# CUHK-AIM-Group/Depth-Aware-Endoscopy-SR

Hardware: AMD Instinct MI355X
Metric: LR frames/sec fwd+bwd at x8 (128x160 LR) (higher is better)
Workload: dtype f32; 1 GPU; Kvasir x8 synthetic, batch=16 per GPU, fp32, DepthNet nb=16 nf=64 L=256 K=10 (BASELINE.json configs[1]); step = fwd + L1 + dynamic loss + bwd + Adam; global_batch=16, scale=8, parallelism=dp1, mode=train, device=cuda, full=False, hip_graph=False

## Files before the change

depth-aware-endoscopy-sr_amd/csrc/bf16.h:

```cpp
#pragma once
#include "dasr_common.h"

typedef __bf16 bf16_t;
typedef __bf16 bf16x8 __attribute__((ext_vector_type(8)));
typedef __bf16 bf16x4 __attribute__((ext_vector_type(4)));
typedef short s16x4 __attribute__((ext_vector_type(4)));

#ifdef DASR_HIPEMU
static inline bf16_t dasr_f2bf(float f) {
    unsigned u;
    memcpy(&u, &f, 4);
    u = (u + 0x7FFFu + ((u >> 16) & 1u)) >> 16;
    unsigned short h = (unsigned short)u;
    bf16_t r;
    memcpy(&r, &h, 2);
    return r;
}
static inline float dasr_bf2f(bf16_t b) {
    unsigned short h;
    memcpy(&h, &b, 2);
    unsigned u = (unsigned)h << 16;
    float f;
    memcpy(&f, &u, 4);
    return f;
// ... 81 lines not shown
#ifdef DASR_HIPEMU
    const hipemu_s16x4 r = hipemu_ds_read_tr16_b64((const void*)p);
#else
    const s16x4 r = __builtin_amdgcn_ds_read_tr16_b64_v4i16((s16x4 __attribute__((address_space(3)))*)p);
#endif
    bf16x4 v;
    __builtin_memcpy(&v, &r, 8);
    return v;
}

typedef unsigned u32x4_t __attribute__((ext_vector_type(4)));
#define DASR_OOB 0x80000000u
#ifdef DASR_HIPEMU
struct BufRsrc {
    const char* base;
    size_t bytes;
};
static inline BufRsrc dasr_make_rsrc(const void* p, size_t bytes) { return BufRsrc{(const char*)p, bytes}; }
static inline u32x4_t dasr_buffer_load16(const BufRsrc& r, unsigned off) {
    u32x4_t v = {0u, 0u, 0u, 0u};
    if ((size_t)off + 16 <= r.bytes) memcpy(&v, r.base + off, 16);
    return v;
}
#else
typedef __amdgpu_buffer_rsrc_t BufRsrc;
__device__ __forceinline__ BufRsrc dasr_make_rsrc(const void* p, size_t bytes) {
    return __builtin_amdgcn_make_buffer_rsrc((void*)p, 0, (int)bytes, 0x00020000);
}
__device__ __forceinline__ u32x4_t dasr_buffer_load16(BufRsrc r, unsigned off) {
    return __builtin_amdgcn_raw_buffer_load_b128(r, (int)off, 0, 0);
}
#endif
```

depth-aware-endoscopy-sr_amd/csrc/conv9_split.hip:

```cpp
#include "bf16.h"
#include "conv_kernels.h"

typedef _Float16 h16_t;
typedef _Float16 h16x8 __attribute__((ext_vector_type(8)));
typedef _Float16 h16x4 __attribute__((ext_vector_type(4)));

#define S9_TH 8

struct Conv9SplitArgs {
    const float* x;
    const float* w;
    const float* bias;
    const float* dy;
    void* out;
    const float* xmax;
    const float* dmax;
    const float* wmax;
    int B, H, W, Cin, Cout;
    int accumulate, P, ntiles;
};

__device__ __forceinline__ float s9_amax_share(const float* buf) {
    float m = 0.f;
    if (buf) {
        int n;
        memcpy(&n, buf, 4);
        for (int i = threadIdx.x; i < n; i += blockDim.x) m = fmaxf(m, buf[1 + i]);
    }
#pragma unroll
    for (int o = 32; o > 0; o >>= 1) m = fmaxf(m, __shfl_xor(m, o));
    return m;
}
__host__ __device__ static inline int s9_scale_exp(float m) {
    unsigned u;
    memcpy(&u, &m, 4);
    int k = 14 - ((int)((u >> 23) & 0xffu) - 127);
    return k < -60 ? -60 : (k > 60 ? 60 : k);
}
__host__ __device__ static inline float s9_pow2(int k) {
    const unsigned u = (unsigned)(127 + k) << 23;
    float f;
    memcpy(&f, &u, 4);
// ... 178 lines not shown
            h16_t h0, h1;
            s9_split(8 * p8 + j < KK ? src[j] : 0.f, sd, h0, h1);
            o0[j] = h0; o1[j] = h1;
        }
        *(h16x8*)(sE0 + (row * S9_TQ + px) * EST + 8 * p8) = o0;
        *(h16x8*)(sE1 + (row * S9_TQ + px) * EST + 8 * p8) = o1;
    }
}
constexpr int S9_NDYE = (S9_TH + 8) * S9_DYW, S9_NDI = (S9_NDYE + 511) / 512;
__device__ __forceinline__ void s9_fetch_dy(const Conv9SplitArgs& a, int b, int y0, int x0, int tid, float (&vdy)[S9_NDI]) {
    const int rowf = (S9_TQ + 8) * a.Cout;
#pragma unroll
    for (int u = 0; u < S9_NDI; ++u) {
        const int idx = tid + 512 * u;
        const int f = idx % S9_DYW, ry = idx / S9_DYW;
        const int gy = y0 - 4 + ry, gx = x0 - 4 + f / a.Cout, co = f % a.Cout;
        const bool ok = idx < S9_NDYE && f < rowf && gy >= 0 && gy < a.H && gx >= 0 && gx < a.W;
        const size_t o = ok ? (((size_t)b * a.H + gy) * a.W + gx) * a.Cout + co : 0;
        const float v = a.dy[o];
        vdy[u] = ok ? v : 0.f;
    }
}

__global__ void __launch_bounds__(512) k_conv9_dgrad_split(Conv9SplitArgs a) {
    DASR_DYN_SMEM(smem);
    constexpr int EST = 40;
    constexpr int NE = (S9_TH + 8) * S9_TQ * EST;
    h16_t* sE0 = (h16_t*)smem;
    h16_t* sE1 = sE0 + NE;
    h16_t* sW0 = sE1 + NE;
    h16_t* sW1 = sW0 + 9 * 32 * EST;
    float* sDy = (float*)(sW1 + 9 * 32 * EST);
    float* s_red = sDy + S9_NDYE;
    const int tid = threadIdx.x, lane = tid & 63, wv = tid >> 6, li = lane & 31, lh = lane >> 5;
    const int tiles_x = (a.W + S9_TQ - 1) / S9_TQ, tiles_y = (a.H + S9_TH - 1) / S9_TH;
    const int total = tiles_x * tiles_y * a.B;
    const int n0 = blockIdx.y * 32;
    const int KK = 9 * a.Cout;
    int kd, kw_;
    s9_scales(a.dmax, a.wmax, s_red, kd, kw_);
    const float sd = s9_pow2(kd), sw = s9_pow2(kw_), inv = s9_pow2(-(kd + kw_));
    {
        float wq[18];
#pragma unroll
        for (int u = 0; u < 18; ++u) {
            const int e = tid + 512 * u, kp = e & 31, ci = (e >> 5) & 31, kh = e >> 10;
            const int kq = kp < KK ? kp : 0, kw = 8 - kq / a.Cout, co = kq % a.Cout;
            const float v = a.w[(((size_t)kh * 9 + kw) * a.Cin + n0 + ci) * a.Cout + co];
            wq[u] = kp < KK ? v : 0.f;
        }
#pragma unroll
        for (int u = 0; u < 18; ++u) {
            const int e = tid + 512 * u, kp = e & 31, ci = (e >> 5) & 31, kh = e >> 10;
            h16_t h0, h1;
            s9_split(wq[u], sw, h0, h1);
            sW0[(kh * 32 + ci) * EST + kp] = h0;
            sW1[(kh * 32 + ci) * EST + kp] = h1;
        }
    }
    float vdy[S9_NDI];
    auto origin = [&](int tile, int& b, int& x0, int& y0) {
        b = tile / (tiles_x * tiles_y);
        const int tt = tile - b * (tiles_x * tiles_y);
        x0 = (tt % tiles_x) * S9_TQ;
        y0 = (tt / tiles_x) * S9_TH;
    };
    int tile = blockIdx.x;
    if (tile < total) {
        int b, x0, y0;
        origin(tile, b, x0, y0);
        s9_fetch_dy(a, b, y0, x0, tid, vdy);
    }
    for (; tile < total; tile += gridDim.x) {
        int b, x0, y0;
        origin(tile, b, x0, y0);
        __syncthreads();
#pragma unroll
        for (int u = 0; u < S9_NDI; ++u) {
            const int idx = tid + 512 * u;
            if (idx < S9_NDYE) sDy[idx] = vdy[u];
        }
        __syncthreads();
        {
            int nb, nx0, ny0;
            origin(tile + (int)gridDim.x < total ? tile + (int)gridDim.x : tile, nb, nx0, ny0);
            s9_fetch_dy(a, nb, ny0, nx0, tid, vdy);
        }
        s9_build_E<EST>(a, sDy, sE0, sE1, sd, tid);
        __syncthreads();
        f32x16 acc;
#pragma unroll
        for (int r = 0; r < 16; ++r) acc[r] = 0.f;
#pragma unroll
        for (int kh = 0; kh < 9; ++kh)
#pragma unroll
            for (int q = 0; q < 2; ++q) {
                const int wo = (kh * 32 + li) * EST + 16 * q + 8 * lh;
                const h16x8 B0 = *(const h16x8*)(sW0 + wo), B1 = *(const h16x8*)(sW1 + wo);
                const int eo = ((wv - kh + 8) * S9_TQ + li) * EST + 16 * q + 8 * lh;
                const h16x8 A0 = *(const h16x8*)(sE0 + eo), A1 = *(const h16x8*)(sE1 + eo);
                acc = s9_mma(A0, A1, B0, B1, acc);
            }
        float* dx = (float*)a.out;
        const int gy = y0 + wv;
        if (gy < a.H) {
#pragma unroll
            for (int g = 0; g < 16; ++g) {
                const int gx = x0 + (g & 3) + 8 * (g >> 2) + 4 * lh;
                if (gx >= a.W) continue;
                const size_t o = (((size_t)b * a.H + gy) * a.W + gx) * a.Cin + n0 + li;
                float v = acc[g] * inv;
                if (a.accumulate) v += dx[o];
                dx[o] = v;
            }
        }
    }
}

__device__ __forceinline__ h16x4 s9_read_tr16(const h16_t* p) {
    const bf16x4 r = lds_read_tr16((const bf16_t*)p);
    h16x4 v;
    __builtin_memcpy(&v, &r, 8);
    return v;
}
__global__ void __launch_bounds__(512) k_conv9_wgrad_split(Conv9SplitArgs a) {
    DASR_DYN_SMEM(smem);
    constexpr int EST = 32;
    constexpr int NX = S9_TH * S9_TQ * 32, NE = (S9_TH + 8) * S9_TQ * EST;
    h16_t* sX0 = (h16_t*)smem;
    h16_t* sX1 = sX0 + NX;
    h16_t* sE0 = sX1 + NX;
    h16_t* sE1 = sE0 + NE;
    float* sDy = (float*)(sE1 + NE);
    float* s_red = sDy + S9_NDYE;
    const int tid = threadIdx.x, lane = tid & 63, wv = DASR_UNIFORM((int)(tid >> 6)), li = lane & 31, lh = lane >> 5;
    const int tiles_x = (a.W + S9_TQ - 1) / S9_TQ, tiles_y = (a.H + S9_TH - 1) / S9_TH;
    const int ci0 = blockIdx.x * 32;
    int kx, kd;
    s9_scales(a.xmax, a.dmax, s_red, kx, kd);
// ... 98 lines not shown
    const float* p = slabs + (size_t)(ci / 32) * (9 * 32 * 32) + (kh * 32 + (ci & 31)) * 32 + np;
    const int s0 = blockIdx.y * per_y;
    const int s1 = s0 + per_y < nslabs ? s0 + per_y : nslabs;
    float acc = 0.f;
    for (int s = s0; s < s1; ++s) acc += p[(size_t)s * cgroups * (9 * 32 * 32)];
    atomicAdd(&dw[i], acc);
}

bool conv9_split_supported(const ConvGeom& g) {
    return conv9_mfma_supported(g) && (g.Cin / 16) * 9 * 32 * S9F_ST * 2 * 2 + (S9_TH + 8) * S9F_TQ * S9F_ST * 2 * 2 + 128 <= 160 * 1024 &&
           (size_t)g.H * g.W * g.Cin * sizeof(float) < ((size_t)1 << 31);
}
int conv9_split_fwd(const ConvGeom& g, const float* x, const float* xmax, const float* w, const float* wmax, const float* bias,
                    float* y, void* stream) {
    Conv9SplitArgs a{x, w, bias, nullptr, y, xmax, nullptr, wmax, g.B, g.H, g.W, g.Cin, g.Cout, 0, 0, 0};
    const int TWO = S9F_TQ - 8;
    const int tiles = ((g.W + TWO - 1) / TWO) * ((g.H + S9_TH - 1) / S9_TH) * g.B;
    const size_t lds = sizeof(h16_t) * (size_t)(2 * (S9_TH + 8) * S9F_TQ * S9F_ST + 2 * (g.Cin / 16) * 9 * 32 * S9F_ST) + 128;
    const int cap = (dasr_get_conv_bf16_impl() & 3) == 2 ? 3 : 256;
    a.P = (tiles >= 256 && cap == 256 && (dasr_get_conv_bf16_impl() & 4096) == 0) ? 1 : 0;
    DASR_LAUNCH(k_conv9_fwd_split, dim3(tiles < cap ? tiles : cap), dim3(512), lds, stream, a);
    DASR_RETURN_LAUNCH_STATUS();
}
int conv9_split_dgrad(const ConvGeom& g, const float* dconv, const float* dmax, const float* w, const float* wmax, float* dx,
                      int accumulate, void* stream) {
    Conv9SplitArgs a{nullptr, w, nullptr, dconv, dx, nullptr, dmax, wmax, g.B, g.H, g.W, g.Cin, g.Cout, accumulate, 0, 0};
    const int tiles = ((g.W + S9_TQ - 1) / S9_TQ) * ((g.H + S9_TH - 1) / S9_TH) * g.B;
    const size_t lds = sizeof(h16_t) * (size_t)(2 * (S9_TH + 8) * S9_TQ * 40 + 2 * 9 * 32 * 40) + sizeof(float) * (size_t)(S9_NDYE + 32);
    int per = 256 / (g.Cin / 32) > 0 ? 256 / (g.Cin / 32) : 1;
    if ((dasr_get_conv_bf16_impl() & 3) == 2) per = 3;
    DASR_LAUNCH(k_conv9_dgrad_split, dim3(tiles < per ? tiles : per, g.Cin / 32), dim3(512), lds, stream, a);
    DASR_RETURN_LAUNCH_STATUS();
}
static void conv9_split_wgrad_plan(const ConvGeom& g, int& ntiles, int& P) {
    ntiles = g.B * ((g.H + S9_TH - 1) / S9_TH) * ((g.W + S9_TQ - 1) / S9_TQ);
    P = 256 / (g.Cin / 32);
    if ((dasr_get_conv_bf16_impl() & 3) == 2) P = 3;
    if (P > ntiles) P = ntiles;
    if (P < 1) P = 1;
}
size_t conv9_split_wgrad_workspace(const ConvGeom& g) {
    const int ntiles = g.B * ((g.H + S9_TH - 1) / S9_TH) * ((g.W + S9_TQ - 1) / S9_TQ);
    int P = 256 / (g.Cin / 32);
    if (P > ntiles) P = ntiles;
    if (P < 1) P = 1;
    return sizeof(float) * (size_t)P * 8 * (g.Cin / 32) * 9 * 32 * 32;
}
int conv9_split_wgrad(const ConvGeom& g, const float* x, const float* xmax, const float* dconv, const float* dmax, float* dw,
                      void* workspace, void* stream) {
    int ntiles, P;
    conv9_split_wgrad_plan(g, ntiles, P);
    Conv9SplitArgs a{x, nullptr, nullptr, dconv, workspace, xmax, dmax, nullptr, g.B, g.H, g.W, g.Cin, g.Cout, 0, P, ntiles};
    const size_t lds = sizeof(h16_t) * (size_t)(2 * S9_TH * S9_TQ * 32 + 2 * (S9_TH + 8) * S9_TQ * 32) +
                       sizeof(float) * (size_t)(S9_NDYE + 32);
    DASR_LAUNCH(k_conv9_wgrad_split, dim3(g.Cin / 32, P), dim3(512), lds, stream, a);
// ... 6 lines not shown
    DASR_RETURN_LAUNCH_STATUS();
}

extern "C" int dasr_conv9_split_supported(int H, int W, int Cin, int Cout) {
    ConvGeom g{1, H, W, Cin, H, W, Cout, 9, 9, 1, 4, 0};
    return (H > 0 && W > 0 && Cin > 0 && Cout > 0 && conv9_split_supported(g)) ? 1 : 0;
}
extern "C" int dasr_conv9_fwd_split2(const float* x, const float* xmax, const float* w_hwio, const float* wmax, const float* bias,
                                     float* y, int B, int H, int W, int Cin, int Cout, void* stream) {
    DASR_CHECK_PTR(x); DASR_CHECK_PTR(xmax); DASR_CHECK_PTR(w_hwio); DASR_CHECK_PTR(wmax); DASR_CHECK_PTR(y);
    DASR_CHECK_SHAPE(B > 0);
    if (!dasr_conv9_split_supported(H, W, Cin, Cout)) return DASR_E_UNSUPPORTED;
    ConvGeom g{B, H, W, Cin, H, W, Cout, 9, 9, 1, 4, 0};
    return conv9_split_fwd(g, x, xmax, w_hwio, wmax, bias, y, stream);
}
extern "C" int dasr_conv9_dgrad_split2(const float* dconv, const float* dmax, const float* w_hwio, const float* wmax, float* dx,
                                       int accumulate, int B, int H, int W, int Cin, int Cout, void* stream) {
    DASR_CHECK_PTR(dconv); DASR_CHECK_PTR(dmax); DASR_CHECK_PTR(w_hwio); DASR_CHECK_PTR(wmax); DASR_CHECK_PTR(dx);
    DASR_CHECK_SHAPE(B > 0);
    if (!dasr_conv9_split_supported(H, W, Cin, Cout)) return DASR_E_UNSUPPORTED;
    ConvGeom g{B, H, W, Cin, H, W, Cout, 9, 9, 1, 4, 0};
    return conv9_split_dgrad(g, dconv, dmax, w_hwio, wmax, dx, accumulate, stream);
}
extern "C" size_t dasr_conv9_wgrad_split2_workspace(int B, int H, int W, int Cin, int Cout) {
    if (B <= 0 || !dasr_conv9_split_supported(H, W, Cin, Cout)) return 0;
    ConvGeom g{B, H, W, Cin, H, W, Cout, 9, 9, 1, 4, 0};
    return conv9_split_wgrad_workspace(g);
}
extern "C" int dasr_conv9_wgrad_split2(const float* x, const float* xmax, const float* dconv, const float* dmax, float* dw_hwio,
                                       float* dbias, void* workspace, size_t workspace_bytes, int B, int H, int W, int Cin,
                                       int Cout, void* stream) {
    DASR_CHECK_PTR(x); DASR_CHECK_PTR(xmax); DASR_CHECK_PTR(dconv); DASR_CHECK_PTR(dmax); DASR_CHECK_PTR(dw_hwio);
    DASR_CHECK_PTR(workspace);
    DASR_CHECK_SHAPE(B > 0);
    if (!dasr_conv9_split_supported(H, W, Cin, Cout)) return DASR_E_UNSUPPORTED;
    if (workspace_bytes < dasr_conv9_wgrad_split2_workspace(B, H, W, Cin, Cout)) return DASR_E_WORKSPACE;
    ConvGeom g{B, H, W, Cin, H, W, Cout, 9, 9, 1, 4, 0};
    int rc = conv9_split_wgrad(g, x, xmax, dconv, dmax, dw_hwio, workspace, stream);
    if (rc) return rc;
    if (dbias) rc = conv_colsum(dconv, dbias, (size_t)B * H * W, Cout, stream);
    return rc;
}
```

depth-aware-endoscopy-sr_amd/csrc/conv_kernels.h:

```cpp
#pragma once
#include "dasr_common.h"
#include "bf16.h"

struct ConvGeom {
    int B, H, W, Cin, Ho, Wo, Cout, KH, KW, stride, pad, transposed;
};

__host__ __device__ __forceinline__ size_t conv_out_index(const ConvGeom& g, int b, int oy, int ox, int co, int ps_r) {
    if (ps_r <= 1) return (((size_t)b * g.Ho + oy) * g.Wo + ox) * g.Cout + co;
    int rr = ps_r * ps_r;
    int c = co / rr, i = (co / ps_r) % ps_r, j = co % ps_r;
    return (((size_t)b * g.Ho * ps_r + (size_t)oy * ps_r + i) * ((size_t)g.Wo * ps_r) + (size_t)ox * ps_r + j) *
               (g.Cout / rr) + c;
}

int conv_direct_fwd(const ConvGeom& g, const float* x, const float* w, const float* bias, const float* residual,
                    float* y, int act, int ps_r, void* stream);
int conv_epilogue_bwd(const ConvGeom& g, const float* dy, const float* y, float* dconv, int act, int ps_r,
                      void* stream, float* amax = nullptr);
int conv_direct_dgrad(const ConvGeom& g, const float* dconv, const float* w, float* dx, int accumulate, void* stream);
int conv_direct_wgrad(const ConvGeom& g, const float* x, const float* dconv, float* dw, void* stream);
int conv_colsum(const float* m, float* out, size_t rows, int C, void* stream);

bool conv_mfma_supported(const ConvGeom& g);
// ... 44 lines not shown
int conv_bf16_dgrad(const ConvGeom& g, const bf16_t* dconv, const bf16_t* w, bf16_t* dx, int accumulate, void* stream);
size_t conv_bf16_wgrad_workspace(const ConvGeom& g);
int conv_bf16_wgrad(const ConvGeom& g, const bf16_t* x, const bf16_t* dconv, float* dw, float* dbias, void* workspace,
                    void* stream);
bool conv_bf16_v2_supported(int H, int W, int Cin, int Cout, int ps_r, bool has_residual, bool accumulate);
int conv_bf16_v2_fwd(const ConvGeom& g, const bf16_t* x, const bf16_t* w, const float* bias, const bf16_t* residual,
                     bf16_t* y, int act, int ps_r, void* stream);
int conv_bf16_v2_dgrad(const ConvGeom& g, const bf16_t* dconv, const bf16_t* w, bf16_t* dx, int accumulate, void* stream);
int conv_epilogue_bwd_bf16(const ConvGeom& g, const bf16_t* dy, const bf16_t* y, bf16_t* dconv, int act, int ps_r,
                           void* stream);
int conv_c1_fwd_bf16(const ConvGeom& g, const float* x, const float* w, const float* bias, bf16_t* y, int act, void* stream);
int conv_c1_wgrad_bf16(const ConvGeom& g, const float* x, const bf16_t* dy, const bf16_t* yact, int act, float* dw,
                       float* dbias, void* stream);
int conv9_bf16_fwd(const ConvGeom& g, const bf16_t* x, const float* w, const float* bias, float* y, void* stream);
int conv9_bf16_dgrad(const ConvGeom& g, const float* dconv, const float* w, bf16_t* dx, int accumulate, void* stream);
size_t conv9_bf16_wgrad_workspace(const ConvGeom& g);
int conv9_bf16_wgrad(const ConvGeom& g, const bf16_t* x, const float* dconv, float* dw, void* workspace, void* stream);

bool conv9_split_supported(const ConvGeom& g);
int conv9_split_fwd(const ConvGeom& g, const float* x, const float* xmax, const float* w, const float* wmax, const float* bias,
                    float* y, void* stream);
int conv9_split_dgrad(const ConvGeom& g, const float* dconv, const float* dmax, const float* w, const float* wmax, float* dx,
                      int accumulate, void* stream);
size_t conv9_split_wgrad_workspace(const ConvGeom& g);
int conv9_split_wgrad(const ConvGeom& g, const float* x, const float* xmax, const float* dconv, const float* dmax, float* dw,
                      void* workspace, void* stream);
```

depth-aware-endoscopy-sr_amd/graph.py:

```python
import math

import torch

from . import ops
from .tape import Tape, Var, accum


FUSE_DGRAD_ACT = False

SIDE_STREAM = True
import os as _os
import threading as _threading
TAIL_WGRAD_SIDE = False
FUSE_INSTNORM_STATS = False
ENCODER_S2D = True
SPLIT_BF16 = True
SPLIT_WGRAD = True
SPLIT_PIECES = 2
FUSE_AMAX = True
SPLIT_CONV9 = True
SPLIT_MIN_PIXELS = 1 << 14
WGRAD_STREAM = False
_SIDE = {}
_SIDE_LOCK = _threading.Lock()


def _side_stream(device, which="branch"):
    key = (str(device), which)
    with _SIDE_LOCK:
        if key not in _SIDE:
            _SIDE[key] = torch.cuda.Stream(device=device, priority=-1)
# ... 260 lines not shown
    elif (SPLIT_BF16 and SPLIT_PIECES == 2 and SPLIT_CONV9 and f32 and w.data.dtype == torch.float32 and stride == 1 and pad == 4
          and not transposed and tuple(w.data.shape[1:3]) == (9, 9) and act == ops.ACT_NONE and ps_r == 1 and residual is None
          and x.data.shape[0] * x.data.shape[1] * x.data.shape[2] >= SPLIT_MIN_PIXELS
          and ops.conv9_split_supported(x.data.shape[1], x.data.shape[2], w.data.shape[3], w.data.shape[4])):
        if w.split is None:
            w.split = ("c9", _folded(tape, ("c9max", "@%x" % w.data.data_ptr()), [w.data], lambda: ops.absmax(w.data[0])))
            if w.pack is not None:
                tape.prepack.note_split(w.pack, w.split)
        y = ops.conv9_fwd_split2(x.data, _amax(x), w.data, w.split[1], bias.data if bias is not None else None)
    else:
        am = want_amax(tape, x.data) if (f32 and x.data.shape[3] in (1, 3) and ps_r == 1) else None
        y = ops.conv2d_fwd(x.data, w.data, bias.data if bias is not None else None,
                           residual.data if residual is not None else None, stride, pad, transposed, act, ps_r, out_dtype,
                           amax=am)
    needs = x.requires_grad or w.requires_grad or (bias is not None and bias.requires_grad) or \
        (residual is not None and residual.requires_grad)
    out = Var(y, needs)
    out.stats = stats
    x.uses += 1
    if residual is not None:
        residual.uses += 1
    if (act != ops.ACT_NONE or ps_r > 1) and residual is None:
        out.epilogue = (act, ps_r)
    KH, KW, Cin, Cout = w.data.shape[1:]
    wshape = (KH, KW, Cin, Cout)
    B, H, W_, _ = x.data.shape
    Ho, Wo = ops.conv_out_hw(H, W_, KH, KW, stride, pad, transposed)

    def bwd():
        if out.grad is None:
            return
        dy = out.grad
        out.grad = None
        if out.grad_event is not None:
            torch.cuda.current_stream().wait_event(out.grad_event)
            dy.record_stream(torch.cuda.current_stream())
        if not x.requires_grad and residual is None and ps_r == 1 and act != ops.ACT_NONE:
            dw, db = ops.conv2d_wgrad_act(x.data, dy, y, wshape, act, stride, pad, transposed,
                                          want_bias=bias is not None)
            accum(w, dw)
            if bias is not None:
                accum(bias, db)
            return
        if out.grad_is_preact:
            dconv = dy
        elif act != ops.ACT_NONE or ps_r > 1:
# ... 21 lines not shown
                cur = torch.cuda.current_stream()
                ready = cur.record_event()
                if ws not in tape.side_streams:
                    tape.side_streams.append(ws)
                with torch.cuda.stream(ws):
                    ws.wait_event(ready)
                    dconv.record_stream(ws)
                    dw, db = ops.conv2d_wgrad(x.data, dconv, wshape, stride, pad, transposed,
                                              want_bias=bias is not None)
                    done = ws.record_event()
                w.grad_event = done
                if bias is not None:
                    bias.grad_event = done
            accum(w, dw)
            if bias is not None:
                accum(bias, db)
        if x.requires_grad:
            if (FUSE_DGRAD_ACT and f32 and x.grad is None and x.uses == 1 and x.epilogue is not None and
                    ops.conv2d_dgrad_act_supported(x.data.shape, w.data, dconv.shape, stride, pad, transposed,
                                                   x.epilogue[1])):
                x.grad = ops.conv2d_dgrad_act(dconv, w.data, x.data, x.epilogue[0], x.epilogue[1], stride, pad,
                                              transposed)
                x.grad_is_preact = True
            elif _is_c9(w):
                if dmax is None:
                    dmax = _amax_t(dconv)
                x.grad = ops.conv9_dgrad_split2(dconv, dmax, w.data, w.split[1], x.data.shape, out=x.grad)
            elif isinstance(w.split, tuple):
                if dmax is None:
                    dmax = _amax_t(dconv)
                x.grad = ops.conv3x3_dgrad_split2(dconv, dmax, w.split, x.data.shape, out=x.grad)
            elif w.split is not None:
                if x.grad is None:
                    x.grad = ops.conv3x3_dgrad_split(dconv, w.split, x.data.shape)
                else:
                    ops.conv3x3_dgrad_split(dconv, w.split, x.data.shape, out=x.grad)
            elif x.grad is None:
                x.grad = ops.conv2d_dgrad(dconv, w.data, x.data.shape, stride, pad, transposed, out_dtype=x.data.dtype)
            else:
                ops.conv2d_dgrad(dconv, w.data, x.data.shape, stride, pad, transposed, out=x.grad)
        if residual is not None:
            accum(residual, dconv)

    tape.record(bwd)
    return out

# ... 438 lines not shown
```

depth-aware-endoscopy-sr_amd/ops.py:

```python
import ctypes

import torch

from . import _lib

ACT_NONE, ACT_RELU, ACT_LRELU = 0, 1, 2
IN_EPS = 1e-5


BF16 = torch.bfloat16


def _p(t, allow_none=False):
    return _lib.ptr(t, allow_none)


def _pa(t, allow_none=False):
    if t is None:
        return _lib.ptr(t, allow_none)
    return _lib.ptr(t, allow_none, dtype=t.dtype if t.dtype in (torch.float32, BF16) else torch.float32)


def _is_bf(*ts):
    kinds = {t.dtype for t in ts if t is not None}
# ... 510 lines not shown
def conv9_split_supported(H, W, Cin, Cout):
    return bool(_lib.get().dasr_conv9_split_supported(H, W, Cin, Cout))


def conv9_fwd_split2(x, xmax, w, wmax, bias):
    B, H, W, Cin = x.shape
    Cout = w.shape[4]
    y = empty((B, H, W, Cout), x)
    _call("dasr_conv9_fwd_split2", _p(x), _p(xmax), _p(w), _p(wmax), _p(bias, True), _p(y), B, H, W, Cin, Cout)
    return y


def conv9_dgrad_split2(dconv, dmax, w, wmax, x_shape, out=None):
    B, H, W, Cin = x_shape
    Cout = dconv.shape[3]
    acc = out is not None
    if out is None:
        out = empty(tuple(x_shape), dconv)
    drop_amax(out)
    _call("dasr_conv9_dgrad_split2", _p(dconv), _p(dmax), _p(w), _p(wmax), _p(out), 1 if acc else 0, B, H, W, Cin, Cout)
    return out


def conv9_wgrad_split2(x, xmax, dconv, dmax, want_bias=True):
    B, H, W, Cin = x.shape
    Cout = dconv.shape[3]
    nbytes = int(_lib.get().dasr_conv9_wgrad_split2_workspace(B, H, W, Cin, Cout))
    ws = torch.empty((max(1, (nbytes + 3) // 4),), dtype=torch.float32, device=x.device)
    dw = empty((9, 9, Cin, Cout), x)
    db = empty((Cout,), x) if want_bias else None
    _call("dasr_conv9_wgrad_split2", _p(x), _p(xmax), _p(dconv), _p(dmax), _p(dw), _p(db, True), _p(ws), nbytes, B, H, W, Cin, Cout)
    return dw, db


def conv2d_fwd_stats(x, w, bias):
    B, H, W, Cin = x.shape
    KH, KW, Cin2, Cout = w.shape[1:]
    assert (KH, KW) == (3, 3) and Cin2 == Cin
    y = empty((B, H, W, Cout), x)
    mean = empty((B, Cout), x)
    var = empty((B, Cout), x)
    nbytes = int(_lib.get().dasr_conv2d_fwd_stats_workspace(B, H, W, Cin, Cout))
    ws = torch.empty((max(1, (nbytes + 3) // 4),), dtype=torch.float32, device=x.device)
    _call("dasr_conv2d_fwd_stats", _p(x), _p(w), _p(bias, True), _p(y), _p(mean), _p(var), _p(ws), nbytes, B, H, W, Cin,
          Cout)
    return y, mean, var
# ... 174 lines not shown
```

depth-aware-endoscopy-sr_amd/tape.py:

```python
from . import ops


class Var:
    __slots__ = ("data", "grad", "requires_grad", "name", "uses", "epilogue", "grad_is_preact", "event",
                 "grad_event", "stats", "split", "amax", "pack")

    def __init__(self, data, requires_grad=False, name=None):
        self.data = data
        self.grad = None
        self.requires_grad = requires_grad
        self.name = name
        self.uses = 0
        self.epilogue = None
        self.grad_is_preact = False
        self.event = None
        self.grad_event = None
        self.stats = None
        self.split = None
        self.amax = None
        self.pack = None

    @property
    def shape(self):
        return self.data.shape


class Tape:

    def __init__(self, enabled=True, act_dtype=None):
        import torch
        self.enabled = enabled
        self.act_dtype = act_dtype if act_dtype is not None else torch.float32
        self.nodes = []
        self._stream = None
        self.side_streams = []
        self.fold_cache = None
# ... 59 lines not shown
```

include/dasr.h:

```cpp
#ifndef DASR_H
#define DASR_H

#include <stddef.h>
#include <stdint.h>

#ifdef __cplusplus
extern "C" {
#endif

#define DASR_OK 0
#define DASR_E_NULL (-1)
#define DASR_E_SHAPE (-2)
#define DASR_E_UNSUPPORTED (-3)
#define DASR_E_WORKSPACE (-4)

#define DASR_ACT_NONE 0
#define DASR_ACT_RELU 1
#define DASR_ACT_LRELU02 2

int dasr_version(void);
const char* dasr_error_string(int code);
int dasr_is_device_build(void);

int dasr_nchw_to_nhwc(const float* src, float* dst, int B, int C, int H, int W, void* stream);
// ... 62 lines not shown
size_t dasr_conv3x3_split2_weights_bytes(int Cin, int Cout);
int dasr_conv3x3_split2_weights(const float* w_packed, const float* wmax, unsigned short* w_split, int Cin, int Cout,
                                void* stream);
typedef struct dasr_split_job {
    const float* w_packed; const float* wmax; unsigned short* w_split;
    int Cin, Cout, wg_begin, reserved;
} dasr_split_job;
int dasr_conv3x3_split2_weights_slabs(int Cin, int Cout);
int dasr_conv3x3_split2_weights_multi(const dasr_split_job* jobs_host, const dasr_split_job* jobs_device, int njobs, void* stream);
int dasr_conv3x3_fwd_split2(const float* x, const float* xmax, const unsigned short* w_split, const float* wmax,
                            const float* bias, const float* residual, float* y, float* y_amax, int B, int H, int W, int Cin,
                            int Cout, int act, int ps_r, void* stream);
int dasr_conv3x3_dgrad_split2(const float* dconv, const float* dmax, const unsigned short* w_split, const float* wmax,
                              float* dx, int accumulate, int B, int H, int W, int Cin, int Cout, void* stream);
int dasr_conv3x3_wgrad_split2(const float* x, const float* xmax, const float* dconv, const float* dmax, float* dw_hwio,
                              float* dbias, void* workspace, size_t workspace_bytes, int B, int H, int W, int Cin, int Cout,
                              void* stream);

int dasr_conv9_split_supported(int H, int W, int Cin, int Cout);
int dasr_conv9_fwd_split2(const float* x, const float* xmax, const float* w_hwio, const float* wmax, const float* bias, float* y,
                          int B, int H, int W, int Cin, int Cout, void* stream);
int dasr_conv9_dgrad_split2(const float* dconv, const float* dmax, const float* w_hwio, const float* wmax, float* dx,
                            int accumulate, int B, int H, int W, int Cin, int Cout, void* stream);
size_t dasr_conv9_wgrad_split2_workspace(int B, int H, int W, int Cin, int Cout);
int dasr_conv9_wgrad_split2(const float* x, const float* xmax, const float* dconv, const float* dmax, float* dw_hwio, float* dbias,
                            void* workspace, size_t workspace_bytes, int B, int H, int W, int Cin, int Cout, void* stream);

size_t dasr_instnorm_stats_workspace(int B, int HW, int C);
int dasr_instnorm_stats(const float* x, float* mean, float* var, void* workspace, size_t workspace_bytes, int B, int HW,
                        int C, void* stream);

int dasr_dynk_fwd(const float* st, const float* A_w, const float* A_b, const float* W_gamma, const float* W_beta,
                  float* stp, float* D, int B, int K, int L, int C, void* stream);
int dasr_dynk_bwd(const float* dD, const float* st, const float* stp, const float* A_w, const float* W_gamma,
                  const float* W_beta, float* dW_gamma, float* dW_beta, float* dA_w, float* dA_b, float* dst,
                  float* dstp, int B, int K, int L, int C, void* stream);

int dasr_mask_compress(const float* mask, unsigned char* region, int* onehot_flag, int B, int K, int H, int W,
                       void* stream);
int dasr_sean_fwd(const float* t, const float* mean, const float* var, const float* gb2, const float* mask,
                  const unsigned char* region, const int* onehot_flag, const float* D, const float* bias_gamma, const float* bias_beta, const float* alpha_gamma,
                  const float* alpha_beta, const float* residual, float* out, float* out_amax, int relu, int B, int H,
                  int W, int C, int K, float eps, void* stream);
size_t dasr_sean_bwd_workspace(int B, int H, int W, int C, int K);
int dasr_sean_bwd(const float* dout, const float* out, const float* t, const float* mean, const float* var,
                  const float* gb2, const float* mask, const unsigned char* region, const int* onehot_flag,
// ... 90 lines not shown
```

Measured before the change: 250.1 frames/s.

## Fuse activation and pixel-shuffle backward into 9x9 split dgrad kernel, retile for occupancy

Rewrites the 9x9 split-fp16 dgrad kernel to use 256-thread workgroups with two per CU, a narrower tile, XOR-swizzled unpadded LDS, dy staged as pre-split halves, a funnel-shift E build, and software-pipelined MFMA operand loads. Adds a fused variant that applies the activation derivative and the pixel-shuffle inverse in the epilogue, writes the pre-activation gradient directly and records the amax. This removes a separate activation-backward and pixel-unshuffle pass plus its memory round trip on the upsampler path. The fused path requires even H/W and ps_r=2 and relies on buffer loads with an OOB offset for edge handling.

```diff
diff --git a/depth-aware-endoscopy-sr_amd/csrc/bf16.h b/depth-aware-endoscopy-sr_amd/csrc/bf16.h
--- a/depth-aware-endoscopy-sr_amd/csrc/bf16.h
+++ b/depth-aware-endoscopy-sr_amd/csrc/bf16.h
@@ -127,6 +127,17 @@
     if ((size_t)off + 16 <= r.bytes) memcpy(&v, r.base + off, 16);
     return v;
 }
+static inline float dasr_buffer_load4f(const BufRsrc& r, unsigned off) {
+    float v = 0.f;
+    if ((size_t)off + 4 <= r.bytes) memcpy(&v, r.base + off, 4);
+    return v;
+}
+static inline void dasr_buffer_store4f(const BufRsrc& r, unsigned off, float v) {
+    if ((size_t)off + 4 <= r.bytes) memcpy(const_cast<char*>(r.base) + off, &v, 4);
+}
+static inline void dasr_buffer_store16f(const BufRsrc& r, unsigned off, float4 v) {
+    if ((size_t)off + 16 <= r.bytes) memcpy(const_cast<char*>(r.base) + off, &v, 16);
+}
 #else
 typedef __amdgpu_buffer_rsrc_t BufRsrc;
 __device__ __forceinline__ BufRsrc dasr_make_rsrc(const void* p, size_t bytes) {
@@ -135,4 +146,13 @@
 __device__ __forceinline__ u32x4_t dasr_buffer_load16(BufRsrc r, unsigned off) {
     return __builtin_amdgcn_raw_buffer_load_b128(r, (int)off, 0, 0);
 }
+__device__ __forceinline__ float dasr_buffer_load4f(BufRsrc r, unsigned off) {
+    return __builtin_bit_cast(float, __builtin_amdgcn_raw_buffer_load_b32(r, (int)off, 0, 0));
+}
+__device__ __forceinline__ void dasr_buffer_store4f(BufRsrc r, unsigned off, float v) {
+    __builtin_amdgcn_raw_buffer_store_b32(__builtin_bit_cast(unsigned, v), r, (int)off, 0, 0);
+}
+__device__ __forceinline__ void dasr_buffer_store16f(BufRsrc r, unsigned off, float4 v) {
+    __builtin_amdgcn_raw_buffer_store_b128(__builtin_bit_cast(u32x4_t, v), r, (int)off, 0, 0);
+}
 #endif
diff --git a/depth-aware-endoscopy-sr_amd/csrc/conv9_split.hip b/depth-aware-endoscopy-sr_amd/csrc/conv9_split.hip
--- a/depth-aware-endoscopy-sr_amd/csrc/conv9_split.hip
+++ b/depth-aware-endoscopy-sr_amd/csrc/conv9_split.hip
@@ -18,6 +18,9 @@
     const float* wmax;
     int B, H, W, Cin, Cout;
     int accumulate, P, ntiles;
+    const float* xact;
+    float* amax;
+    int act;
 };
 
 __device__ __forceinline__ float s9_amax_share(const float* buf) {
@@ -242,99 +245,210 @@
     }
 }
 
-__global__ void __launch_bounds__(512) k_conv9_dgrad_split(Conv9SplitArgs a) {
+#define S9D_TQ 16
+#define S9D_DYW ((S9D_TQ + 8) * 3 + 8)
+constexpr int S9D_NDYE = (S9_TH + 8) * S9D_DYW, S9D_NDI = S9D_NDYE / 256;
+static_assert(S9D_NDI * 256 == S9D_NDYE, "dy tile: whole trips of 256 threads");
+constexpr size_t S9D_LDS = sizeof(h16_t) * (size_t)(2 * (S9_TH + 8) * S9D_TQ * 32 + 2 * 9 * 32 * 32) + sizeof(float) * (size_t)(S9D_NDYE + 32);
+static_assert(2 * S9D_LDS <= 160 * 1024, "two workgroups per CU");
+typedef unsigned u32a_t __attribute__((may_alias));
+typedef unsigned u32x4a_t __attribute__((ext_vector_type(4), may_alias));
+__device__ __forceinline__ unsigned s9d_fsh(unsigned lo, unsigned hi, unsigned bits) {
+#if DASR_DEVICE_BUILD
+    return __builtin_amdgcn_alignbit(hi, lo, bits);
+#else
+    return (unsigned)((((unsigned long long)hi << 32) | lo) >> bits);
+#endif
+}
+template <bool FUSE>
+__global__ void __launch_bounds__(256, 2) k_conv9_dgrad_split(Conv9SplitArgs a) {
     DASR_DYN_SMEM(smem);
-    constexpr int EST = 40;
-    constexpr int NE = (S9_TH + 8) * S9_TQ * EST;
+    constexpr int NE = (S9_TH + 8) * S9D_TQ * 32;
     h16_t* sE0 = (h16_t*)smem;
     h16_t* sE1 = sE0 + NE;
     h16_t* sW0 = sE1 + NE;
-    h16_t* sW1 = sW0 + 9 * 32 * EST;
-    float* sDy = (float*)(sW1 + 9 * 32 * EST);
-    float* s_red = sDy + S9_NDYE;
+    h16_t* sW1 = sW0 + 9 * 32 * 32;
+    h16_t* sH0 = sW1 + 9 * 32 * 32;
+    h16_t* sH1 = sH0 + S9D_NDYE;
+    float* s_red = (float*)(sH1 + S9D_NDYE);
     const int tid = threadIdx.x, lane = tid & 63, wv = tid >> 6, li = lane & 31, lh = lane >> 5;
-    const int tiles_x = (a.W + S9_TQ - 1) / S9_TQ, tiles_y = (a.H + S9_TH - 1) / S9_TH;
+    const int tiles_x = (a.W + S9D_TQ - 1) / S9D_TQ, tiles_y = (a.H + S9_TH - 1) / S9_TH;
     const int total = tiles_x * tiles_y * a.B;
     const int n0 = blockIdx.y * 32;
     const int KK = 9 * a.Cout;
     int kd, kw_;
     s9_scales(a.dmax, a.wmax, s_red, kd, kw_);
     const float sd = s9_pow2(kd), sw = s9_pow2(kw_), inv = s9_pow2(-(kd + kw_));
-    {
+#pragma unroll 1
+    for (int h = 0; h < 2; ++h) {
         float wq[18];
 #pragma unroll
         for (int u = 0; u < 18; ++u) {
-            const int e = tid + 512 * u, kp = e & 31, ci = (e >> 5) & 31, kh = e >> 10;
+            const int e = tid + 256 * (18 * h + u), kp = e & 31, ci = (e >> 5) & 31, kh = e >> 10;
             const int kq = kp < KK ? kp : 0, kw = 8 - kq / a.Cout, co = kq % a.Cout;
             const float v = a.w[(((size_t)kh * 9 + kw) * a.Cin + n0 + ci) * a.Cout + co];
             wq[u] = kp < KK ? v : 0.f;
         }
 #pragma unroll
         for (int u = 0; u < 18; ++u) {
-            const int e = tid + 512 * u, kp = e & 31, ci = (e >> 5) & 31, kh = e >> 10;
+            const int e = tid + 256 * (18 * h + u), kp = e & 31, ci = (e >> 5) & 31, kh = e >> 10;
             h16_t h0, h1;
             s9_split(wq[u], sw, h0, h1);
-            sW0[(kh * 32 + ci) * EST + kp] = h0;
-            sW1[(kh * 32 + ci) * EST + kp] = h1;
-        }
-    }
-    float vdy[S9_NDI];
+            const int o = (kh * 32 + ci) * 32 + 8 * ((kp >> 3) ^ ((ci >> 2) & 3)) + (kp & 7);
+            sW0[o] = h0;
+            sW1[o] = h1;
+        }
+    }
+    int dyr[S9D_NDI], dyx[S9D_NDI], dyo[S9D_NDI];
+#pragma unroll
+    for (int u = 0; u < S9D_NDI; ++u) {
+        const int idx = tid + 256 * u, f = idx % S9D_DYW, ry = idx / S9D_DYW;
+        dyr[u] = ry - 4;
+        dyx[u] = f < (S9D_TQ + 8) * a.Cout ? f / a.Cout - 4 : (1 << 28);
+        dyo[u] = (dyr[u] * a.W - 4) * a.Cout + f;
+    }
+    float vdy[S9D_NDI];
     auto origin = [&](int tile, int& b, int& x0, int& y0) {
         b = tile / (tiles_x * tiles_y);
         const int tt = tile - b * (tiles_x * tiles_y);
-        x0 = (tt % tiles_x) * S9_TQ;
+        x0 = (tt % tiles_x) * S9D_TQ;
         y0 = (tt / tiles_x) * S9_TH;
     };
+    auto fetch = [&](int b, int y0, int x0) {
+        const BufRsrc rd = dasr_make_rsrc(a.dy + (size_t)b * a.H * a.W * a.Cout, (size_t)a.H * a.W * a.Cout * sizeof(float));
+        const int base = (y0 * a.W + x0) * a.Cout;
+#pragma unroll
+        for (int u = 0; u < S9D_NDI; ++u) {
+            const bool ok = (unsigned)(y0 + dyr[u]) < (unsigned)a.H && (unsigned)(x0 + dyx[u]) < (unsigned)a.W;
+            vdy[u] = dasr_buffer_load4f(rd, ok ? (unsigned)((base + dyo[u]) * (int)sizeof(float)) : DASR_OOB);
+        }
+    };
+    const int prow = 2 * wv + (li >> 4), pcol = li & 15;
+    const int asw = (pcol >> 2) & 3, bsw = (li >> 2) & 3;
+    const int p8 = tid & 3, epx = (tid >> 2) & 15, r0 = tid >> 6;
+    const int es = a.Cout * epx + 8 * p8;
+    const unsigned ebits = (es & 1) * 16;
+    const int esrc = r0 * S9D_DYW + (es & ~1), edst = (r0 * S9D_TQ + epx) * 32 + 8 * (p8 ^ ((epx >> 2) & 3));
+    unsigned em[4];
+#pragma unroll
+    for (int d = 0; d < 4; ++d) em[d] = (8 * p8 + 2 * d < KK ? 0xffffu : 0u) | (8 * p8 + 2 * d + 1 < KK ? 0xffff0000u : 0u);
+    const size_t img = (size_t)a.H * a.W * a.Cin;
+    const unsigned rowst = (unsigned)(a.W * a.Cin) * sizeof(float), pixst = (unsigned)a.Cin * sizeof(float);
+    const float dneg = a.act == DASR_ACT_RELU ? 0.f : (a.act == DASR_ACT_LRELU02 ? 0.2f : 1.f);
+    float om = 0.f;
     int tile = blockIdx.x;
     if (tile < total) {
         int b, x0, y0;
         origin(tile, b, x0, y0);
-        s9_fetch_dy(a, b, y0, x0, tid, vdy);
+        fetch(b, y0, x0);
     }
     for (; tile < total; tile += gridDim.x) {
         int b, x0, y0;
         origin(tile, b, x0, y0);
-        __syncthreads();
-#pragma unroll
-        for (int u = 0; u < S9_NDI; ++u) {
-            const int idx = tid + 512 * u;
-            if (idx < S9_NDYE) sDy[idx] = vdy[u];
-        }
-        __syncthreads();
+#pragma unroll
+        for (int u = 0; u < S9D_NDI; ++u) {
+            h16_t h0, h1;
+            s9_split(vdy[u], sd, h0, h1);
+            sH0[tid + 256 * u] = h0;
+            sH1[tid + 256 * u] = h1;
+        }
+        DASR_LDS_BARRIER();
         {
             int nb, nx0, ny0;
             origin(tile + (int)gridDim.x < total ? tile + (int)gridDim.x : tile, nb, nx0, ny0);
-            s9_fetch_dy(a, nb, ny0, nx0, tid, vdy);
-        }
-        s9_build_E<EST>(a, sDy, sE0, sE1, sd, tid);
-        __syncthreads();
+            fetch(nb, ny0, nx0);
+        }
+        unsigned xoff[4];
+        const bool rowok = y0 + 2 * wv < a.H;
+#pragma unroll
+        for (int cp = 0; cp < 4; ++cp) {
+            const int cx = x0 + 4 * lh + 2 * (cp & 1) + 8 * (cp >> 1);
+            xoff[cp] = (rowok && cx < a.W) ? (unsigned)((((y0 + 2 * wv) * a.W + cx) * a.Cin + n0 + li) * (int)sizeof(float)) : DASR_OOB;
+        }
+        auto pix_off = [&](int g) {
+            const unsigned o = xoff[((g >> 2) & 1) * 2 + ((g & 3) >> 1)] + (g >> 3) * rowst + (g & 1) * pixst;
+            if (FUSE) return o;
+            return (y0 + 2 * wv + (g >> 3) < a.H && x0 + 4 * lh + (g & 3) + 8 * ((g >> 2) & 1) < a.W) ? o : DASR_OOB;
+        };
+        float xa[16];
+        if (FUSE) {
+            const BufRsrc rx = dasr_make_rsrc(a.xact + (size_t)b * img, img * sizeof(float));
+#pragma unroll
+            for (int g = 0; g < 16; ++g) xa[g] = dasr_buffer_load4f(rx, pix_off(g));
+        }
+#pragma unroll
+        for (int i = 0; i < (S9_TH + 8) / 4; ++i) {
+            const u32a_t* s0 = (const u32a_t*)(sH0 + esrc + i * 4 * S9D_DYW);
+            const u32a_t* s1 = (const u32a_t*)(sH1 + esrc + i * 4 * S9D_DYW);
+            u32x4_t o0, o1;
+#pragma unroll
+            for (int d = 0; d < 4; ++d) {
+                o0[d] = s9d_fsh(s0[d], s0[d + 1], ebits) & em[d];
+                o1[d] = s9d_fsh(s1[d], s1[d + 1], ebits) & em[d];
+            }
+            *(u32x4a_t*)(sE0 + edst + i * 4 * S9D_TQ * 32) = o0;
+            *(u32x4a_t*)(sE1 + edst + i * 4 * S9D_TQ * 32) = o1;
+        }
+        DASR_LDS_BARRIER();
         f32x16 acc;
 #pragma unroll
         for (int r = 0; r < 16; ++r) acc[r] = 0.f;
-#pragma unroll
-        for (int kh = 0; kh < 9; ++kh)
-#pragma unroll
-            for (int q = 0; q < 2; ++q) {
-                const int wo = (kh * 32 + li) * EST + 16 * q + 8 * lh;
-                const h16x8 B0 = *(const h16x8*)(sW0 + wo), B1 = *(const h16x8*)(sW1 + wo);
-                const int eo = ((wv - kh + 8) * S9_TQ + li) * EST + 16 * q + 8 * lh;
-                const h16x8 A0 = *(const h16x8*)(sE0 + eo), A1 = *(const h16x8*)(sE1 + eo);
-                acc = s9_mma(A0, A1, B0, B1, acc);
-            }
-        float* dx = (float*)a.out;
-        const int gy = y0 + wv;
-        if (gy < a.H) {
-#pragma unroll
-            for (int g = 0; g < 16; ++g) {
-                const int gx = x0 + (g & 3) + 8 * (g >> 2) + 4 * lh;
-                if (gx >= a.W) continue;
-                const size_t o = (((size_t)b * a.H + gy) * a.W + gx) * a.Cin + n0 + li;
-                float v = acc[g] * inv;
-                if (a.accumulate) v += dx[o];
-                dx[o] = v;
-            }
-        }
-    }
+        {
+            const int wb = li * 32, eb = ((prow + 8) * S9D_TQ + pcol) * 32;
+            const int pw0 = 8 * (lh ^ bsw), pw1 = 8 * ((2 + lh) ^ bsw), pe0 = 8 * (lh ^ asw), pe1 = 8 * ((2 + lh) ^ asw);
+            h16x8 A0 = *(const h16x8*)(sE0 + eb + pe0), A1 = *(const h16x8*)(sE1 + eb + pe0);
+            h16x8 B0 = *(const h16x8*)(sW0 + wb + pw0), B1 = *(const h16x8*)(sW1 + wb + pw0);
+            DASR_SCHED_BARRIER();
+#pragma unroll
+            for (int s = 0; s < 18; ++s) {
+                const h16x8 a0 = A0, a1 = A1, b0 = B0, b1 = B1;
+                if (s + 1 < 18) {
+                    const int kh = (s + 1) >> 1, q = (s + 1) & 1;
+                    const int wo = wb + kh * 32 * 32 + (q ? pw1 : pw0), eo = eb - kh * S9D_TQ * 32 + (q ? pe1 : pe0);
+                    A0 = *(const h16x8*)(sE0 + eo); A1 = *(const h16x8*)(sE1 + eo);
+                    B0 = *(const h16x8*)(sW0 + wo); B1 = *(const h16x8*)(sW1 + wo);
+                }
+                acc = s9_mma(a0, a1, b0, b1, acc);
+                if (s + 1 < 18) DASR_SCHED_GROUP(0x100, 4);
+                DASR_SCHED_GROUP(0x8, 3);
+            }
+            DASR_SCHED_BARRIER();
+        }
+        if (FUSE) {
+            const BufRsrc rp = dasr_make_rsrc((float*)a.out + (size_t)b * img, img * sizeof(float));
+            const int Wc = a.W >> 1, cy = (y0 >> 1) + wv;
+#pragma unroll
+            for (int j = 0; j < 4; ++j) {
+                const int g = 2 * (j & 1) + 4 * (j >> 1);
+                const int cx = x0 + 4 * lh + 2 * (j & 1) + 8 * (j >> 1);
+                const bool ok = xoff[j] != DASR_OOB;
+                float4 o;
+                o.x = acc[g] * inv * (xa[g] > 0.f ? 1.f : dneg);
+                o.y = acc[g + 1] * inv * (xa[g + 1] > 0.f ? 1.f : dneg);
+                o.z = acc[g + 8] * inv * (xa[g + 8] > 0.f ? 1.f : dneg);
+                o.w = acc[g + 9] * inv * (xa[g + 9] > 0.f ? 1.f : dneg);
+                dasr_buffer_store16f(rp, ok ? (unsigned)(((cy * Wc + (cx >> 1)) * (4 * a.Cin) + 4 * (n0 + li)) * (int)sizeof(float)) : DASR_OOB, o);
+                om = fmaxf(om, ok ? dasr_amax4(0.f, o) : 0.f);
+            }
+        } else {
+            const BufRsrc ro = dasr_make_rsrc((float*)a.out + (size_t)b * img, img * sizeof(float));
+            if (a.accumulate) {
+                float old[16];
+#pragma unroll
+                for (int g = 0; g < 16; ++g) old[g] = dasr_buffer_load4f(ro, pix_off(g));
+#pragma unroll
+                for (int g = 0; g < 16; ++g) {
+                    float v = acc[g] * inv;
+                    v += old[g];
+                    dasr_buffer_store4f(ro, pix_off(g), v);
+                }
+            } else {
+#pragma unroll
+                for (int g = 0; g < 16; ++g) dasr_buffer_store4f(ro, pix_off(g), acc[g] * inv);
+            }
+        }
+    }
+    if (FUSE && a.amax) dasr_amax_commit(a.amax, om, s_red, dasr_flat_wg(), dasr_flat_nwg());
 }
 
 __device__ __forceinline__ h16x4 s9_read_tr16(const h16_t* p) {
@@ -479,15 +593,26 @@
     DASR_LAUNCH(k_conv9_fwd_split, dim3(tiles < cap ? tiles : cap), dim3(512), lds, stream, a);
     DASR_RETURN_LAUNCH_STATUS();
 }
+static int conv9_split_dgrad_launch(const ConvGeom& g, Conv9SplitArgs& a, bool fuse, void* stream) {
+    const int tiles = ((g.W + S9D_TQ - 1) / S9D_TQ) * ((g.H + S9_TH - 1) / S9_TH) * g.B;
+    int per = 512 / (g.Cin / 32) > 0 ? 512 / (g.Cin / 32) : 1;
+    if ((dasr_get_conv_bf16_impl() & 3) == 2) per = 3;
+    const dim3 grid(tiles < per ? tiles : per, g.Cin / 32);
+    if (fuse)
+        DASR_LAUNCH(k_conv9_dgrad_split<true>, grid, dim3(256), S9D_LDS, stream, a);
+    else
+        DASR_LAUNCH(k_conv9_dgrad_split<false>, grid, dim3(256), S9D_LDS, stream, a);
+    DASR_RETURN_LAUNCH_STATUS();
+}
 int conv9_split_dgrad(const ConvGeom& g, const float* dconv, const float* dmax, const float* w, const float* wmax, float* dx,
                       int accumulate, void* stream) {
     Conv9SplitArgs a{nullptr, w, nullptr, dconv, dx, nullptr, dmax, wmax, g.B, g.H, g.W, g.Cin, g.Cout, accumulate, 0, 0};
-    const int tiles = ((g.W + S9_TQ - 1) / S9_TQ) * ((g.H + S9_TH - 1) / S9_TH) * g.B;
-    const size_t lds = sizeof(h16_t) * (size_t)(2 * (S9_TH + 8) * S9_TQ * 40 + 2 * 9 * 32 * 40) + sizeof(float) * (size_t)(S9_NDYE + 32);
-    int per = 256 / (g.Cin / 32) > 0 ? 256 / (g.Cin / 32) : 1;
-    if ((dasr_get_conv_bf16_impl() & 3) == 2) per = 3;
-    DASR_LAUNCH(k_conv9_dgrad_split, dim3(tiles < per ? tiles : per, g.Cin / 32), dim3(512), lds, stream, a);
-    DASR_RETURN_LAUNCH_STATUS();
+    return conv9_split_dgrad_launch(g, a, false, stream);
+}
+int conv9_split_dgrad_act(const ConvGeom& g, const float* dconv, const float* dmax, const float* w, const float* wmax,
+                          const float* x_act, float* dprev, float* amax, int act, void* stream) {
+    Conv9SplitArgs a{nullptr, w, nullptr, dconv, dprev, nullptr, dmax, wmax, g.B, g.H, g.W, g.Cin, g.Cout, 0, 0, 0, x_act, amax, act};
+    return conv9_split_dgrad_launch(g, a, true, stream);
 }
 static void conv9_split_wgrad_plan(const ConvGeom& g, int& ntiles, int& P) {
     ntiles = g.B * ((g.H + S9_TH - 1) / S9_TH) * ((g.W + S9_TQ - 1) / S9_TQ);
@@ -540,6 +665,17 @@
     ConvGeom g{B, H, W, Cin, H, W, Cout, 9, 9, 1, 4, 0};
     return conv9_split_dgrad(g, dconv, dmax, w_hwio, wmax, dx, accumulate, stream);
 }
+extern "C" int dasr_conv9_dgrad_act_split2(const float* dconv, const float* dmax, const float* w_hwio, const float* wmax,
+                                           const float* x_act, float* dprev, float* amax, int B, int H, int W, int Cin, int Cout,
+                                           int act, int ps_r, void* stream) {
+    DASR_CHECK_PTR(dconv); DASR_CHECK_PTR(dmax); DASR_CHECK_PTR(w_hwio); DASR_CHECK_PTR(wmax); DASR_CHECK_PTR(x_act); DASR_CHECK_PTR(dprev);
+    DASR_CHECK_SHAPE(B > 0);
+    if (ps_r != 2 || (H & 1) || (W & 1) || !(act == DASR_ACT_NONE || act == DASR_ACT_RELU || act == DASR_ACT_LRELU02) ||
+        !dasr_conv9_split_supported(H, W, Cin, Cout))
+        return DASR_E_UNSUPPORTED;
+    ConvGeom g{B, H, W, Cin, H, W, Cout, 9, 9, 1, 4, 0};
+    return conv9_split_dgrad_act(g, dconv, dmax, w_hwio, wmax, x_act, dprev, amax, act, stream);
+}
 extern "C" size_t dasr_conv9_wgrad_split2_workspace(int B, int H, int W, int Cin, int Cout) {
     if (B <= 0 || !dasr_conv9_split_supported(H, W, Cin, Cout)) return 0;
     ConvGeom g{B, H, W, Cin, H, W, Cout, 9, 9, 1, 4, 0};
diff --git a/depth-aware-endoscopy-sr_amd/csrc/conv_kernels.h b/depth-aware-endoscopy-sr_amd/csrc/conv_kernels.h
--- a/depth-aware-endoscopy-sr_amd/csrc/conv_kernels.h
+++ b/depth-aware-endoscopy-sr_amd/csrc/conv_kernels.h
@@ -90,6 +90,8 @@
                     float* y, void* stream);
 int conv9_split_dgrad(const ConvGeom& g, const float* dconv, const float* dmax, const float* w, const float* wmax, float* dx,
                       int accumulate, void* stream);
+int conv9_split_dgrad_act(const ConvGeom& g, const float* dconv, const float* dmax, const float* w, const float* wmax,
+                          const float* x_act, float* dprev, float* amax, int act, void* stream);
 size_t conv9_split_wgrad_workspace(const ConvGeom& g);
 int conv9_split_wgrad(const ConvGeom& g, const float* x, const float* xmax, const float* dconv, const float* dmax, float* dw,
                       void* workspace, void* stream);
diff --git a/depth-aware-endoscopy-sr_amd/graph.py b/depth-aware-endoscopy-sr_amd/graph.py
--- a/depth-aware-endoscopy-sr_amd/graph.py
+++ b/depth-aware-endoscopy-sr_amd/graph.py
@@ -7,6 +7,7 @@
 
 
 FUSE_DGRAD_ACT = False
+FUSE_C9_DGRAD_ACT = True
 
 SIDE_STREAM = True
 import os as _os
@@ -313,6 +314,7 @@
         residual.uses += 1
     if (act != ops.ACT_NONE or ps_r > 1) and residual is None:
         out.epilogue = (act, ps_r)
+        out.epilogue_split = isinstance(w.split, tuple)
     KH, KW, Cin, Cout = w.data.shape[1:]
     wshape = (KH, KW, Cin, Cout)
     B, H, W_, _ = x.data.shape
@@ -380,6 +382,14 @@
                 x.grad = ops.conv2d_dgrad_act(dconv, w.data, x.data, x.epilogue[0], x.epilogue[1], stride, pad,
                                               transposed)
                 x.grad_is_preact = True
+            elif (_is_c9(w) and FUSE_C9_DGRAD_ACT and x.grad is None and x.uses == 1 and x.epilogue is not None
+                  and ops.conv9_dgrad_act_supported(x.data.shape, Cout, x.epilogue[0], x.epilogue[1])):
+                if dmax is None:
+                    dmax = _amax_t(dconv)
+                x.grad = ops.conv9_dgrad_act_split2(dconv, dmax, w.data, w.split[1], x.data, x.epilogue[0], x.epilogue[1],
+                                                    amax=want_amax(tape, dconv, (B, H // 2, W_ // 2, 4 * Cin))
+                                                    if x.epilogue_split else None)
+                x.grad_is_preact = True
             elif _is_c9(w):
                 if dmax is None:
                     dmax = _amax_t(dconv)
diff --git a/depth-aware-endoscopy-sr_amd/ops.py b/depth-aware-endoscopy-sr_amd/ops.py
--- a/depth-aware-endoscopy-sr_amd/ops.py
+++ b/depth-aware-endoscopy-sr_amd/ops.py
@@ -556,6 +556,21 @@
     return out
 
 
+def conv9_dgrad_act_supported(x_shape, Cout, act, ps_r):
+    B, H, W, Cin = x_shape
+    return (ps_r == 2 and H % 2 == 0 and W % 2 == 0 and act in (ACT_NONE, ACT_RELU, ACT_LRELU)
+            and conv9_split_supported(H, W, Cin, Cout))
+
+
+def conv9_dgrad_act_split2(dconv, dmax, w, wmax, x_act, act, ps_r, amax=None):
+    B, H, W, Cin = x_act.shape
+    Cout = dconv.shape[3]
+    dprev = empty((B, H // 2, W // 2, 4 * Cin), dconv)
+    _call("dasr_conv9_dgrad_act_split2", _p(dconv), _p(dmax), _p(w), _p(wmax), _p(x_act), _p(dprev), _p(amax, True),
+          B, H, W, Cin, Cout, act, ps_r)
+    return set_amax(dprev, amax)
+
+
 def conv9_wgrad_split2(x, xmax, dconv, dmax, want_bias=True):
     B, H, W, Cin = x.shape
     Cout = dconv.shape[3]
diff --git a/depth-aware-endoscopy-sr_amd/tape.py b/depth-aware-endoscopy-sr_amd/tape.py
--- a/depth-aware-endoscopy-sr_amd/tape.py
+++ b/depth-aware-endoscopy-sr_amd/tape.py
@@ -3,7 +3,7 @@
 
 class Var:
     __slots__ = ("data", "grad", "requires_grad", "name", "uses", "epilogue", "grad_is_preact", "event",
-                 "grad_event", "stats", "split", "amax", "pack")
+                 "grad_event", "stats", "split", "amax", "pack", "epilogue_split")
 
     def __init__(self, data, requires_grad=False, name=None):
         self.data = data
@@ -12,6 +12,7 @@
         self.name = name
         self.uses = 0
         self.epilogue = None
+        self.epilogue_split = False
         self.grad_is_preact = False
         self.event = None
         self.grad_event = None
diff --git a/include/dasr.h b/include/dasr.h
--- a/include/dasr.h
+++ b/include/dasr.h
@@ -108,6 +108,9 @@
                           int B, int H, int W, int Cin, int Cout, void* stream);
 int dasr_conv9_dgrad_split2(const float* dconv, const float* dmax, const float* w_hwio, const float* wmax, float* dx,
                             int accumulate, int B, int H, int W, int Cin, int Cout, void* stream);
+int dasr_conv9_dgrad_act_split2(const float* dconv, const float* dmax, const float* w_hwio, const float* wmax, const float* x_act,
+                                float* dprev, float* amax, int B, int H, int W, int Cin, int Cout, int act, int ps_r,
+                                void* stream);
 size_t dasr_conv9_wgrad_split2_workspace(int B, int H, int W, int Cin, int Cout);
 int dasr_conv9_wgrad_split2(const float* x, const float* xmax, const float* dconv, const float* dmax, float* dw_hwio, float* dbias,
                             void* workspace, size_t workspace_bytes, int B, int H, int W, int Cin, int Cout, void* stream);
```

New measurement: 257.8 frames/s (median of 6 runs). +3.1%, better.
